# david-macmahon/BLDistributedDataProducts.jl

Hardware: AMD Instinct MI355X
Metric: filterbank GB/s reduced (node) + % HBM roofline, 8-bank 0000 band (higher is better)
Workload: dtype f32

## Files before the change

### bldistributeddataproducts.jl_amd/csrc/bslz4.hip

```cpp
#include <algorithm>
#include <cstring>
#include <vector>

#include "bldp_impl.h"

namespace {

inline uint32_t be32(const uint8_t *p) {
  return (uint32_t)p[0] << 24 | (uint32_t)p[1] << 16 | (uint32_t)p[2] << 8 | p[3];
}
inline uint64_t be64(const uint8_t *p) { return (uint64_t)be32(p) << 32 | be32(p + 4); }

__host__ __device__ inline uint64_t transpose8(uint64_t x) {
  uint64_t t;
  t = (x ^ (x >> 7)) & 0x00AA00AA00AA00AAull;
  x = x ^ t ^ (t << 7);
  t = (x ^ (x >> 14)) & 0x0000CCCC0000CCCCull;
  x = x ^ t ^ (t << 14);
  t = (x ^ (x >> 28)) & 0x00000000F0F0F0F0ull;
  x = x ^ t ^ (t << 28);
  return x;
}

int64_t lz4_block_host(const uint8_t *src, size_t slen, uint8_t *dst, size_t dcap) {
  size_t ip = 0, op = 0;
  while (ip < slen) {
    const uint8_t token = src[ip++];
    size_t lit = token >> 4;
    if (lit == 15) {
      uint8_t b;
      do {
        if (ip >= slen) return -1;
        b = src[ip++];
        lit += b;
      } while (b == 255);
    }
    if (ip + lit > slen || op + lit > dcap) return -1;
    memcpy(dst + op, src + ip, lit);
    ip += lit;
    op += lit;
    if (ip >= slen) break;
    if (ip + 2 > slen) return -1;
    const size_t off = (size_t)src[ip] | (size_t)src[ip + 1] << 8;
    ip += 2;
    size_t ml = token & 15;
    if (ml == 15) {
      uint8_t b;
      do {
        if (ip >= slen) return -1;
        b = src[ip++];
        ml += b;
      } while (b == 255);
    }
    ml += 4;
    if (off == 0 || off > op || op + ml > dcap) return -1;
    for (size_t i = 0; i < ml; ++i) dst[op + i] = dst[op - off + i];
    op += ml;
  }
  return (int64_t)op;
}

void bitunshuffle_host(const uint8_t *planes, uint8_t *out, size_t n, size_t es) {
  const size_t rowb = n / 8;
  for (size_t g = 0; g < rowb; ++g)
    for (size_t j = 0; j < es; ++j) {
      uint64_t x = 0;
      for (int k = 0; k < 8; ++k) x |= (uint64_t)planes[(j * 8 + k) * rowb + g] << (8 * k);
      x = transpose8(x);
      for (int t = 0; t < 8; ++t) out[(8 * g + t) * es + j] = (uint8_t)(x >> (8 * t));
    }
}

struct Task {
  uint64_t src;
  uint64_t dst;
  uint32_t clen;
  uint32_t nelem;
};
constexpr uint32_t RAW = 0xFFFFFFFFu;

struct ChunkDesc {
  uint64_t src, len, dst;
  uint64_t n, block;
  uint32_t nfull, last, tail;
  uint32_t task0;
};

int describe_chunk(const uint8_t *c, uint64_t len, uint64_t src, uint64_t dst, int es,
                   ChunkDesc *d) {
  if (len < 12) return bldp::set_error(BLDP_EINVAL, "bslz4: chunk shorter than its header");
  const uint64_t nb = be64(c);
  const uint32_t bb = be32(c + 8);
  if (nb % es || bb % es || bb == 0 || (bb / es) % 8 || bb > (1u << 24))
    return bldp::set_error(BLDP_EINVAL, "bslz4: bad header (bytes %llu, block %u, elem %d)",
                           (unsigned long long)nb, bb, es);
  d->src = src;
  d->len = len;
  d->dst = dst;
  d->n = nb / es;
  d->block = bb / es;
  d->nfull = (uint32_t)(d->n / d->block);
  uint64_t last = d->n % d->block;
  d->last = (uint32_t)(last - last % 8);
  d->tail = (uint32_t)(d->n - (uint64_t)d->nfull * d->block - d->last);
  return BLDP_OK;
}

inline uint32_t ntasks(const ChunkDesc &d) {
  return d.nfull + (d.last ? 1 : 0) + (d.tail ? 1 : 0);
}

__host__ __device__ inline uint32_t lz4_bound(uint32_t n) { return n + n / 255 + 16; }

__device__ inline uint32_t be32_dev(const uint8_t *p) {
  return (uint32_t)p[0] << 24 | (uint32_t)p[1] << 16 | (uint32_t)p[2] << 8 | p[3];
}

__global__ __launch_bounds__(64) void k_bslz4_plan(const uint8_t *__restrict__ comp,
                                                   const ChunkDesc *__restrict__ chunks,
                                                   int nchunk, int es, uint32_t cap,
                                                   Task *__restrict__ tasks, int *err) {
  const int k = blockIdx.x * 64 + threadIdx.x;
  if (k >= nchunk) return;
  const ChunkDesc d = chunks[k];
  uint64_t pos = d.src + 12, e = 0;
  const uint64_t end = d.src + d.len;
  const uint32_t nblk = d.nfull + (d.last ? 1 : 0);
  for (uint32_t b = 0; b < nblk; ++b) {
    const uint32_t ne = b < d.nfull ? (uint32_t)d.block : d.last;
    if (pos + 4 > end) { atomicOr(err, 2); return; }
    const uint32_t cl = be32_dev(comp + pos);
    if (cl > cap || pos + 4 + cl > end) { atomicOr(err, 2); return; }
    tasks[d.task0 + b] = Task{pos + 4, d.dst + e * es, cl, ne};
    pos += 4 + cl;
    e += ne;
  }
  if (pos + (uint64_t)d.tail * es != end) { atomicOr(err, 4); return; }
  if (d.tail) tasks[d.task0 + nblk] = Task{pos, d.dst + e * es, RAW, d.tail};
}

int plan_chunk(const uint8_t *c, uint64_t len, uint64_t src0, uint64_t dst0, int es,
               std::vector<Task> &tasks, uint64_t *out_bytes, uint32_t *max_block) {
  if (len < 12) return bldp::set_error(BLDP_EINVAL, "bslz4: chunk shorter than its header");
  const uint64_t nb = be64(c);
  const uint32_t bb = be32(c + 8);
  if (nb % es || bb % es || bb == 0 || (bb / es) % 8)
    return bldp::set_error(BLDP_EINVAL, "bslz4: bad header (bytes %llu, block %u, elem %d)",
                           (unsigned long long)nb, bb, es);
  const uint64_t n = nb / es, block = bb / es;
  uint64_t pos = 12, e = 0;
  const uint64_t nfull = n / block;
  uint64_t last = n % block;
  last -= last % 8;
  for (uint64_t k = 0; k < nfull + (last ? 1 : 0); ++k) {
    const uint64_t ne = k < nfull ? block : last;
    if (pos + 4 > len) return bldp::set_error(BLDP_EINVAL, "bslz4: truncated block header");
    const uint32_t cl = be32(c + pos);
    if (cl == RAW || pos + 4 + cl > len)
      return bldp::set_error(BLDP_EINVAL, "bslz4: block %llu overruns the chunk",
                             (unsigned long long)k);
    tasks.push_back(Task{src0 + pos + 4, dst0 + e * es, cl, (uint32_t)ne});
    *max_block = std::max<uint32_t>(*max_block, std::max<uint32_t>(cl, (uint32_t)(ne * es)));
    pos += 4 + cl;
    e += ne;
  }
  const uint64_t tail = n - e;
  if (pos + tail * es != len)
    return bldp::set_error(BLDP_EINVAL, "bslz4: %llu trailing bytes, expected %llu",
                           (unsigned long long)(len - pos), (unsigned long long)(tail * es));
  if (tail) tasks.push_back(Task{src0 + pos, dst0 + e * es, RAW, (uint32_t)tail});
  *out_bytes = nb;
  return BLDP_OK;
}

__global__ __launch_bounds__(64) void k_bslz4(const uint8_t *__restrict__ comp,
                                              const Task *__restrict__ tasks, int ntask,
                                              uint8_t *__restrict__ out, int es, uint32_t cap,
                                              int *err) {
  extern __shared__ uint8_t lds[];
  const int lane = threadIdx.x;
  if (*err & 6) return;
  const Task t = tasks[blockIdx.x];
  if (t.clen == RAW) {
    for (uint32_t i = lane; i < t.nelem * (uint32_t)es; i += 64) out[t.dst + i] = comp[t.src + i];
    return;
  }
  uint8_t *in = lds, *dec = lds + cap;
  const uint32_t clen = t.clen, nbytes = t.nelem * (uint32_t)es;
  if (clen > cap) {
    if (lane == 0) atomicOr(err, 1);
    return;
  }
  for (uint32_t i = lane; i < clen; i += 64) in[i] = comp[t.src + i];
  __syncthreads();
  uint32_t ip = 0, op = 0;
  bool bad = false;
  while (ip < clen) {
    const uint32_t token = in[ip++];
    uint32_t lit = token >> 4;
    if (lit == 15) {
      uint32_t b;
      do {
        if (ip >= clen) { bad = true; break; }
        b = in[ip++];
        lit += b;
      } while (b == 255);
      if (bad) break;
    }
    if (ip + lit > clen || op + lit > nbytes) { bad = true; break; }
    for (uint32_t i = lane; i < lit; i += 64) dec[op + i] = in[ip + i];
    ip += lit;
    op += lit;
    if (ip >= clen) break;
    if (ip + 2 > clen) { bad = true; break; }
    const uint32_t off = (uint32_t)in[ip] | (uint32_t)in[ip + 1] << 8;
    ip += 2;
    uint32_t ml = token & 15;
    if (ml == 15) {
      uint32_t b;
      do {
        if (ip >= clen) { bad = true; break; }
        b = in[ip++];
        ml += b;
      } while (b == 255);
      if (bad) break;
    }
    ml += 4;
    if (off == 0 || off > op || op + ml > nbytes) { bad = true; break; }
    __syncthreads();
    const uint32_t step = off < 64 ? off : 64;
    for (uint32_t r = 0; r < ml; r += step) {
      const uint32_t i = r + lane;
      if (lane < step && i < ml) dec[op + i] = dec[op - off + i];
      __syncthreads();
    }
    op += ml;
  }
  if (bad || op != nbytes) {
    if (lane == 0) atomicOr(err, 1);
    return;
  }
  __syncthreads();
  const uint32_t rowb = t.nelem / 8;
  if (es == 4) {
    for (uint32_t g = lane; g < rowb; g += 64) {
      uint32_t w[8] = {0, 0, 0, 0, 0, 0, 0, 0};
#pragma unroll
      for (int j = 0; j < 4; ++j) {
        uint64_t x = 0;
#pragma unroll
        for (int k = 0; k < 8; ++k) x |= (uint64_t)dec[(j * 8 + k) * rowb + g] << (8 * k);
        x = transpose8(x);
#pragma unroll
        for (int q = 0; q < 8; ++q) w[q] |= (uint32_t)((x >> (8 * q)) & 0xFF) << (8 * j);
      }
      uint32_t *o = reinterpret_cast<uint32_t *>(out + t.dst) + 8 * g;
#pragma unroll
      for (int q = 0; q < 8; ++q) o[q] = w[q];
    }
  } else {
    for (uint32_t g = lane; g < rowb; g += 64)
      for (int j = 0; j < es; ++j) {
        uint64_t x = 0;
        for (int k = 0; k < 8; ++k) x |= (uint64_t)dec[(j * 8 + k) * rowb + g] << (8 * k);
        x = transpose8(x);
        for (int q = 0; q < 8; ++q) out[t.dst + (8 * g + q) * es + j] = (uint8_t)(x >> (8 * q));
      }
  }
}

}

extern "C" {

BLDP_API int bldp_bslz4_info(const void *chunk, size_t nbytes, uint64_t *uncompressed_bytes,
                             uint32_t *block_bytes) {
  if (!chunk || nbytes < 12 || !uncompressed_bytes || !block_bytes)
    return bldp::set_error(BLDP_EINVAL, "bslz4: null pointer or short chunk");
  *uncompressed_bytes = be64((const uint8_t *)chunk);
  *block_bytes = be32((const uint8_t *)chunk + 8);
  return BLDP_OK;
}

BLDP_API int bldp_bslz4_decode_host(const void *chunk, size_t nbytes, int elem_size, void *out,
                                    size_t out_bytes) {
  if (!chunk || (!out && out_bytes) || elem_size <= 0)
    return bldp::set_error(BLDP_EINVAL, "bslz4: bad argument");
  std::vector<Task> tasks;
  uint64_t total = 0;
  uint32_t maxb = 0;
  int rc = plan_chunk((const uint8_t *)chunk, nbytes, 0, 0, elem_size, tasks, &total, &maxb);
  if (rc) return rc;
  if (total != out_bytes)
    return bldp::set_error(BLDP_EINVAL, "bslz4: chunk holds %llu bytes, output has %zu",
                           (unsigned long long)total, out_bytes);
  const uint8_t *c = (const uint8_t *)chunk;
  uint8_t *o = (uint8_t *)out;
  std::vector<uint8_t> dec(maxb);
  for (const Task &t : tasks) {
    const size_t nb = (size_t)t.nelem * elem_size;
    if (t.clen == RAW) {
      memcpy(o + t.dst, c + t.src, nb);
      continue;
    }
    if (lz4_block_host(c + t.src, t.clen, dec.data(), nb) != (int64_t)nb)
      return bldp::set_error(BLDP_EINVAL, "bslz4: corrupt LZ4 block at byte %llu",
                             (unsigned long long)t.src);
    bitunshuffle_host(dec.data(), o + t.dst, t.nelem, elem_size);
  }
  return BLDP_OK;
}

static int decode_launch(int nchunk, const uint8_t *comp_host, const uint8_t *comp_dev,
                         const uint64_t *chunk_off, const uint64_t *chunk_len, int elem_size,
                         uint8_t *out_dev, const uint64_t *out_off, const uint64_t *out_len,
                         int *derr_user, hipStream_t s, int **derr_used,
                         bldp::ScratchLease &lease, uint64_t host_base = 0) {
  if (nchunk < 0 || (nchunk && (!comp_host || !comp_dev || !chunk_off || !chunk_len ||
                                !out_dev || !out_off || !out_len)) ||
      elem_size <= 0 || elem_size > 64)
    return bldp::set_error(BLDP_EINVAL, "bslz4: bad argument");
  if (elem_size == 4 && ((uintptr_t)out_dev & 3))
    return bldp::set_error(BLDP_EINVAL, "bslz4: output must be 4-byte aligned");
  std::vector<ChunkDesc> descs(nchunk);
  uint64_t ntask = 0;
  uint32_t maxbb = 0;
  for (int k = 0; k < nchunk; ++k) {
    if (chunk_off[k] < host_base)
      return bldp::set_error(BLDP_EINVAL, "bslz4: chunk %d below the host staging base", k);
    int rc = describe_chunk(comp_host + (chunk_off[k] - host_base), chunk_len[k], chunk_off[k],
                            out_off[k],
                            elem_size, &descs[k]);
    if (rc) return rc;
    if (descs[k].n * (uint64_t)elem_size != out_len[k])
      return bldp::set_error(BLDP_EINVAL,
                             "bslz4: chunk %d decodes to %llu bytes, its output slot holds %llu",
                             k, (unsigned long long)(descs[k].n * elem_size),
                             (unsigned long long)out_len[k]);
    if (elem_size == 4 && (out_off[k] & 3))
      return bldp::set_error(BLDP_EINVAL, "bslz4: output offsets must be 4-byte aligned");
    descs[k].task0 = (uint32_t)ntask;
    ntask += ntasks(descs[k]);
    if (ntask > INT32_MAX) return bldp::set_error(BLDP_EINVAL, "bslz4: too many blocks");
    maxbb = std::max<uint32_t>(maxbb, (uint32_t)(descs[k].block * elem_size));
  }
  *derr_used = nullptr;
  if (ntask == 0) return BLDP_OK;
  const uint32_t cap = (lz4_bound(maxbb) + 15) & ~15u;
  if ((size_t)cap + (((size_t)maxbb + 15) & ~(size_t)15) > 64 * 1024)
    return bldp::set_error(BLDP_EINVAL, "bslz4: block of %u bytes exceeds the LDS plan", maxbb);
  const size_t dbytes = ((descs.size() * sizeof(ChunkDesc)) + 255) & ~(size_t)255;
  const size_t tbytes = ((ntask * sizeof(Task)) + 255) & ~(size_t)255;
  int rc = bldp::scratch_lease(s, dbytes + tbytes + 256, &lease);
  if (rc) return rc;
  void *ws = lease.ptr;
  ChunkDesc *ddesc = (ChunkDesc *)ws;
  Task *dtask = (Task *)((char *)ws + dbytes);
  int *derr = derr_user ? derr_user : (int *)((char *)ws + dbytes + tbytes);
  if (hipMemcpyAsync(ddesc, descs.data(), descs.size() * sizeof(ChunkDesc),
                     hipMemcpyHostToDevice, s) != hipSuccess ||
      (!derr_user && hipMemsetAsync(derr, 0, sizeof(int), s) != hipSuccess))
    return bldp::set_error(BLDP_EHIP, "bslz4: descriptor upload failed");
  hipLaunchKernelGGL(k_bslz4_plan, dim3((unsigned)((nchunk + 63) / 64)), dim3(64), 0, s,
                     comp_dev, ddesc, nchunk, elem_size, cap, dtask, derr);
  const uint32_t dcap = (maxbb + 15) & ~15u;
  hipLaunchKernelGGL(k_bslz4, dim3((unsigned)ntask), dim3(64), cap + dcap, s, comp_dev, dtask,
                     (int)ntask, out_dev, elem_size, cap, derr);
  hipError_t e = hipGetLastError();
  if (e != hipSuccess) return bldp::set_error(BLDP_EHIP, "bslz4 launch: %s", hipGetErrorString(e));
  *derr_used = derr;
  return BLDP_OK;
}

static int decode_error(int herr) {
  if (herr & 6) return bldp::set_error(BLDP_EINVAL, "bslz4: block table overruns a chunk");
  if (herr) return bldp::set_error(BLDP_EINVAL, "bslz4: corrupt LZ4 block on the device");
  return BLDP_OK;
}

BLDP_API int bldp_bslz4_decode_dev(int nchunk, const uint8_t *comp_host, const uint8_t *comp_dev,
                                   const uint64_t *chunk_off, const uint64_t *chunk_len,
                                   int elem_size, uint8_t *out_dev, const uint64_t *out_off,
                                   const uint64_t *out_len, void *stream) {
  hipStream_t s = (hipStream_t)stream;
  int *derr = nullptr;
  bldp::ScratchLease lease;
  int rc = decode_launch(nchunk, comp_host, comp_dev, chunk_off, chunk_len, elem_size, out_dev,
                         out_off, out_len, nullptr, s, &derr, lease);
  if (rc || !derr) return rc;
  int herr = 0;
  if (hipMemcpyAsync(&herr, derr, sizeof(int), hipMemcpyDeviceToHost, s) != hipSuccess ||
      hipStreamSynchronize(s) != hipSuccess)
    return bldp::set_error(BLDP_EHIP, "bslz4: synchronize failed");
  return decode_error(herr);
}

BLDP_API int bldp_bslz4_decode_dev_async(int nchunk, const uint8_t *comp_host,
                                         const uint8_t *comp_dev, const uint64_t *chunk_off,
                                         const uint64_t *chunk_len, int elem_size,
                                         uint8_t *out_dev, const uint64_t *out_off,
                                         const uint64_t *out_len, int *err_dev, void *stream) {
  if (!err_dev) return bldp::set_error(BLDP_EINVAL, "bslz4: null error word");
  int *derr = nullptr;
  bldp::ScratchLease lease;
  return decode_launch(nchunk, comp_host, comp_dev, chunk_off, chunk_len, elem_size, out_dev,
                       out_off, out_len, err_dev, (hipStream_t)stream, &derr, lease);
}

BLDP_API int bldp_bslz4_error(const int *err_dev, void *stream) {
  if (!err_dev) return bldp::set_error(BLDP_EINVAL, "bslz4: null error word");
  int herr = 0;
  hipStream_t s = (hipStream_t)stream;
  if (hipMemcpyAsync(&herr, err_dev, sizeof(int), hipMemcpyDeviceToHost, s) != hipSuccess ||
      hipStreamSynchronize(s) != hipSuccess)
    return bldp::set_error(BLDP_EHIP, "bslz4: synchronize failed");
  return decode_error(herr);
}

}

int bldp::bslz4_decode_async_at(int nchunk, const uint8_t *comp_host, uint64_t host_base,
                                const uint8_t *comp_dev, const uint64_t *chunk_off,
                                const uint64_t *chunk_len, int elem_size, uint8_t *out_dev,
                                const uint64_t *out_off, const uint64_t *out_len, int *err_dev,
                                hipStream_t s) {
  if (!err_dev) return bldp::set_error(BLDP_EINVAL, "bslz4: null error word");
  int *derr = nullptr;
  bldp::ScratchLease lease;
  return decode_launch(nchunk, comp_host, comp_dev, chunk_off, chunk_len, elem_size, out_dev,
                       out_off, out_len, err_dev, s, &derr, lease, host_base);
}
```

Measured before the change: 7428.

## Widen bslz4 decode to dword LDS staging, literal copies, and bitshuffle output

Reworks the HIP bitshuffle-LZ4 decoder. Compressed input is staged into LDS as aligned dwords using alignbyte funnel shifts, and literal runs are copied as dwords instead of bytes. Match copies now run without a barrier per step, using a lane phase modulo the offset. The bit-unshuffle writes 32 elements per lane with 16-byte stores. Token parsing uses readfirstlane to keep the parse scalar. The aim is to cut byte-granular LDS and global traffic and barrier stalls, at the cost of more complex index math and higher register pressure (32+32 arrays per lane).

```diff
diff --git a/bldistributeddataproducts.jl_amd/csrc/bslz4.hip b/bldistributeddataproducts.jl_amd/csrc/bslz4.hip
--- a/bldistributeddataproducts.jl_amd/csrc/bslz4.hip
+++ b/bldistributeddataproducts.jl_amd/csrc/bslz4.hip
@@ -3,6 +3,7 @@
 #include <vector>
 
 #include "bldp_impl.h"
+#include "bslz4_lanes.h"
 
 namespace {
 
@@ -11,16 +12,7 @@
 }
 inline uint64_t be64(const uint8_t *p) { return (uint64_t)be32(p) << 32 | be32(p + 4); }
 
-__host__ __device__ inline uint64_t transpose8(uint64_t x) {
-  uint64_t t;
-  t = (x ^ (x >> 7)) & 0x00AA00AA00AA00AAull;
-  x = x ^ t ^ (t << 7);
-  t = (x ^ (x >> 14)) & 0x0000CCCC0000CCCCull;
-  x = x ^ t ^ (t << 14);
-  t = (x ^ (x >> 28)) & 0x00000000F0F0F0F0ull;
-  x = x ^ t ^ (t << 28);
-  return x;
-}
+using bslz4::transpose8;
 
 int64_t lz4_block_host(const uint8_t *src, size_t slen, uint8_t *dst, size_t dcap) {
   size_t ip = 0, op = 0;
@@ -177,50 +169,98 @@
                                               const Task *__restrict__ tasks, int ntask,
                                               uint8_t *__restrict__ out, int es, uint32_t cap,
                                               int *err) {
-  extern __shared__ uint8_t lds[];
-  const int lane = threadIdx.x;
+  extern __shared__ uint32_t ldsw[];
+  const uint32_t lane = threadIdx.x;
   if (*err & 6) return;
   const Task t = tasks[blockIdx.x];
   if (t.clen == RAW) {
     for (uint32_t i = lane; i < t.nelem * (uint32_t)es; i += 64) out[t.dst + i] = comp[t.src + i];
     return;
   }
-  uint8_t *in = lds, *dec = lds + cap;
-  const uint32_t clen = t.clen, nbytes = t.nelem * (uint32_t)es;
+  uint32_t *inw = ldsw, *decw = ldsw + cap / 4;
+  uint8_t *in = reinterpret_cast<uint8_t *>(inw), *dec = reinterpret_cast<uint8_t *>(decw);
+  const uint32_t clen = __builtin_amdgcn_readfirstlane(t.clen);
+  const uint32_t nbytes = __builtin_amdgcn_readfirstlane(t.nelem * (uint32_t)es);
   if (clen > cap) {
     if (lane == 0) atomicOr(err, 1);
     return;
   }
-  for (uint32_t i = lane; i < clen; i += 64) in[i] = comp[t.src + i];
+  {
+    const uint8_t *g = comp + t.src;
+    const uint32_t mis = (uint32_t)(reinterpret_cast<uintptr_t>(g) & 3);
+    const uint32_t *gw = reinterpret_cast<const uint32_t *>(g - mis);
+    const uint32_t nw = bslz4::stage_words(clen);
+    for (uint32_t j0 = lane; j0 < nw; j0 += 64 * bslz4::STAGE_BATCH) {
+      uint32_t lo[bslz4::STAGE_BATCH], hi[bslz4::STAGE_BATCH];
+#pragma unroll
+      for (uint32_t u = 0; u < bslz4::STAGE_BATCH; ++u) {
+        const uint32_t j = j0 + 64 * u;
+        lo[u] = j < nw ? gw[j] : 0;
+        hi[u] = j < nw && bslz4::stage_needs_hi(mis, clen, j) ? gw[j + 1] : 0;
+      }
+#pragma unroll
+      for (uint32_t u = 0; u < bslz4::STAGE_BATCH; ++u) {
+        const uint32_t j = j0 + 64 * u;
+        if (j >= nw) break;
+        const uint32_t v = bslz4::funnel(hi[u], lo[u], mis);
+        const uint32_t nb = bslz4::stage_store_bytes(clen, j);
+        if (nb == 4) {
+          inw[j] = v;
+        } else {
+          in[4 * j] = (uint8_t)v;
+          if (nb > 1) in[4 * j + 1] = (uint8_t)(v >> 8);
+          if (nb > 2) in[4 * j + 2] = (uint8_t)(v >> 16);
+        }
+      }
+    }
+  }
   __syncthreads();
+  auto byte_at = [&](uint32_t i) -> uint32_t {
+    return (uint32_t)__builtin_amdgcn_readfirstlane((int)in[i]);
+  };
   uint32_t ip = 0, op = 0;
   bool bad = false;
   while (ip < clen) {
-    const uint32_t token = in[ip++];
+    const uint32_t token = byte_at(ip++);
     uint32_t lit = token >> 4;
     if (lit == 15) {
       uint32_t b;
       do {
         if (ip >= clen) { bad = true; break; }
-        b = in[ip++];
+        b = byte_at(ip++);
         lit += b;
       } while (b == 255);
       if (bad) break;
     }
     if (ip + lit > clen || op + lit > nbytes) { bad = true; break; }
-    for (uint32_t i = lane; i < lit; i += 64) dec[op + i] = in[ip + i];
+    {
+      const uint32_t nw = bslz4::lit_words(op, lit);
+      for (uint32_t k = lane; k < nw; k += 64) {
+        const bslz4::LitWord w = bslz4::lit_word(ip, op, lit, k);
+        const uint32_t lo = w.lo >= 0 ? inw[w.lo] : 0;
+        const uint32_t hi = w.hi >= 0 ? inw[w.hi] : 0;
+        const uint32_t v = bslz4::funnel(hi, lo, w.s);
+        if (w.b1 - w.b0 == 4) {
+          decw[w.dw] = v;
+        } else {
+#pragma unroll
+          for (uint32_t b = 0; b < 4; ++b)
+            if (b >= w.b0 && b < w.b1) dec[4 * w.dw + b] = (uint8_t)(v >> (8 * b));
+        }
+      }
+    }
     ip += lit;
     op += lit;
     if (ip >= clen) break;
     if (ip + 2 > clen) { bad = true; break; }
-    const uint32_t off = (uint32_t)in[ip] | (uint32_t)in[ip + 1] << 8;
+    const uint32_t off = byte_at(ip) | byte_at(ip + 1) << 8;
     ip += 2;
     uint32_t ml = token & 15;
     if (ml == 15) {
       uint32_t b;
       do {
         if (ip >= clen) { bad = true; break; }
-        b = in[ip++];
+        b = byte_at(ip++);
         ml += b;
       } while (b == 255);
       if (bad) break;
@@ -228,11 +268,11 @@
     ml += 4;
     if (off == 0 || off > op || op + ml > nbytes) { bad = true; break; }
     __syncthreads();
-    const uint32_t step = off < 64 ? off : 64;
-    for (uint32_t r = 0; r < ml; r += step) {
-      const uint32_t i = r + lane;
-      if (lane < step && i < ml) dec[op + i] = dec[op - off + i];
-      __syncthreads();
+    const uint32_t stride = bslz4::match_stride(off);
+    uint32_t ph = bslz4::match_phase0(lane, off);
+    for (uint32_t i = lane; i < ml; i += 64) {
+      dec[op + i] = dec[op - off + ph];
+      ph = bslz4::match_advance(ph, stride, off);
     }
     op += ml;
   }
@@ -242,7 +282,24 @@
   }
   __syncthreads();
   const uint32_t rowb = t.nelem / 8;
-  if (es == 4) {
+  if (es == 4 && (rowb & 3) == 0) {
+    uint32_t *o = reinterpret_cast<uint32_t *>(out + t.dst);
+    const bool wide = (reinterpret_cast<uintptr_t>(o) & 15) == 0;
+    for (uint32_t q = lane; q < rowb / 4; q += 64) {
+      uint32_t p[32], e[32];
+#pragma unroll
+      for (uint32_t r = 0; r < 32; ++r) p[r] = decw[bslz4::plane_dword(r, rowb, q)];
+      bslz4::gather32(p, e);
+      if (wide) {
+        uint4 *o4 = reinterpret_cast<uint4 *>(o) + 8 * q;
+#pragma unroll
+        for (int i = 0; i < 8; ++i) o4[i] = make_uint4(e[4 * i], e[4 * i + 1], e[4 * i + 2], e[4 * i + 3]);
+      } else {
+#pragma unroll
+        for (int i = 0; i < 32; ++i) o[32 * q + i] = e[i];
+      }
+    }
+  } else if (es == 4) {
     for (uint32_t g = lane; g < rowb; g += 64) {
       uint32_t w[8] = {0, 0, 0, 0, 0, 0, 0, 0};
 #pragma unroll
diff --git a/bldistributeddataproducts.jl_amd/csrc/bslz4_lanes.h b/bldistributeddataproducts.jl_amd/csrc/bslz4_lanes.h
--- /dev/null
+++ b/bldistributeddataproducts.jl_amd/csrc/bslz4_lanes.h
@@ -0,0 +1,99 @@
+#pragma once
+#include <cstdint>
+
+#if defined(__HIPCC__) || defined(__CUDACC__)
+#define BSLZ4_HD __host__ __device__ inline
+#else
+#define BSLZ4_HD inline
+#endif
+
+namespace bslz4 {
+
+constexpr uint32_t WAVE = 64;
+
+BSLZ4_HD uint64_t transpose8(uint64_t x) {
+  uint64_t t;
+  t = (x ^ (x >> 7)) & 0x00AA00AA00AA00AAull;
+  x = x ^ t ^ (t << 7);
+  t = (x ^ (x >> 14)) & 0x0000CCCC0000CCCCull;
+  x = x ^ t ^ (t << 14);
+  t = (x ^ (x >> 28)) & 0x00000000F0F0F0F0ull;
+  x = x ^ t ^ (t << 28);
+  return x;
+}
+
+BSLZ4_HD uint32_t funnel(uint32_t hi, uint32_t lo, uint32_t s) {
+#if defined(__HIP_DEVICE_COMPILE__)
+  return __builtin_amdgcn_alignbyte(hi, lo, s);
+#else
+  return (uint32_t)((((uint64_t)hi << 32) | lo) >> (8 * s));
+#endif
+}
+
+BSLZ4_HD uint32_t match_phase0(uint32_t lane, uint32_t off) {
+  return lane < off ? lane : lane % off;
+}
+BSLZ4_HD uint32_t match_stride(uint32_t off) { return WAVE % off; }
+BSLZ4_HD uint32_t match_advance(uint32_t phase, uint32_t stride, uint32_t off) {
+  phase += stride;
+  return phase >= off ? phase - off : phase;
+}
+
+constexpr uint32_t STAGE_BATCH = 4;
+BSLZ4_HD uint32_t stage_words(uint32_t clen) { return (clen + 3) >> 2; }
+BSLZ4_HD bool stage_needs_hi(uint32_t mis, uint32_t clen, uint32_t j) {
+  return mis != 0 && 4 * j + 4 < mis + clen;
+}
+BSLZ4_HD uint32_t stage_store_bytes(uint32_t clen, uint32_t j) {
+  const uint32_t left = clen - 4 * j;
+  return left < 4 ? left : 4;
+}
+
+struct LitWord {
+  int32_t lo, hi;
+  uint32_t s;
+  uint32_t dw;
+  uint32_t b0, b1;
+};
+BSLZ4_HD uint32_t lit_words(uint32_t op, uint32_t lit) {
+  return lit ? ((op + lit + 3) >> 2) - (op >> 2) : 0;
+}
+BSLZ4_HD LitWord lit_word(uint32_t ip, uint32_t op, uint32_t lit, uint32_t k) {
+  LitWord w;
+  w.dw = (op >> 2) + k;
+  const int32_t d0 = (int32_t)(4 * w.dw);
+  const int32_t sb = (int32_t)ip + d0 - (int32_t)op;
+  w.s = (uint32_t)sb & 3u;
+  const int32_t sw = (sb - (int32_t)w.s) / 4;
+  const int32_t s0 = (int32_t)ip, s1 = (int32_t)(ip + lit);
+  w.lo = (4 * sw + 3 >= s0 && 4 * sw < s1) ? sw : -1;
+  w.hi = (w.s != 0 && 4 * sw + 7 >= s0 && 4 * sw + 4 < s1) ? sw + 1 : -1;
+  const int32_t e0 = (int32_t)op > d0 ? (int32_t)op : d0;
+  const int32_t e1 = (int32_t)(op + lit) < d0 + 4 ? (int32_t)(op + lit) : d0 + 4;
+  w.b0 = (uint32_t)(e0 - d0);
+  w.b1 = (uint32_t)(e1 - d0);
+  return w;
+}
+
+BSLZ4_HD uint32_t plane_dword(uint32_t p, uint32_t rowb, uint32_t q) {
+  return p * (rowb >> 2) + q;
+}
+BSLZ4_HD void gather32(const uint32_t planes[32], uint32_t elems[32]) {
+#pragma unroll
+  for (int c = 0; c < 4; ++c) {
+    uint32_t w[8] = {0, 0, 0, 0, 0, 0, 0, 0};
+#pragma unroll
+    for (int j = 0; j < 4; ++j) {
+      uint64_t x = 0;
+#pragma unroll
+      for (int k = 0; k < 8; ++k) x |= (uint64_t)((planes[8 * j + k] >> (8 * c)) & 0xFF) << (8 * k);
+      x = transpose8(x);
+#pragma unroll
+      for (int t = 0; t < 8; ++t) w[t] |= (uint32_t)((x >> (8 * t)) & 0xFF) << (8 * j);
+    }
+#pragma unroll
+    for (int t = 0; t < 8; ++t) elems[8 * c + t] = w[t];
+  }
+}
+
+}
```

After: 7428. About the same (-0.0%).
